# generic-ebpf/generic-ebpf

Hardware: AMD Instinct MI355X
Metric: Mpkt/s device-resident (64-insn filter, 64B pkts); achieved HBM GB/s vs peak (higher is better)
Workload: dtype u64; 1 GPU; c4; desc=64-insn classify + array-map lookup, 64 B packets, packets_total=67108864, packets_per_gpu=67108864, packet_bytes=64, prog_slots=553, dprog_entries=122, variant=0, exec=compiled, kernel_layout=staged64, parallelism=dp1, launch=eager, faulted_packets=0

## Files before the change

generic-ebpf_amd/csrc/asm/gen_interp.py:

```python
#!/usr/bin/env python3
import re
import sys
from typing import NamedTuple

from gen_emit import *
from gen_handlers import handler_body
from gen_image import IMAGES, SETTINGS
from gen_jit import entry_reads, jit_templates
from gen_routines import routines


def kernel(img, name, staged, jit=False):
    k = "K%s%s" % ("s" if staged else "g", "j" if jit else "")
    L = [".globl %s" % name, ".p2align 8", ".type %s,@function" % name, "%s:" % name]
    if name == "ebpf_jit_s64" and img.phased and img.slots == 16:
        L += [".globl ebpf_jit_s64w", ".type ebpf_jit_s64w,@function", "ebpf_jit_s64w:"]
    L += ["v_readfirstlane_b32 %s, v0" % s(S_WAVE),
          "s_lshr_b32 %s, %s, 6" % (s(S_WAVE), s(S_WAVE)),
          "s_load_dwordx16 s[%d:%d], %s" % (S_PROG, S_PROG + 15, karg_regs(
              ("prog", S_PROG), ("maps", S_MAPS), ("data", S_DATA), ("offsets", S_OFFS),
              ("off_base", S_OFFBASE), ("ret", S_RET), ("faults", S_FAULTS), ("hist", S_HIST))),
          "s_load_dwordx8 s[%d:%d], %s" % (S_COUNT, S_COUNT + 7, karg_regs(
              ("count", S_COUNT), ("stride", S_STRIDE), ("start", S_START), ("nmaps", S_NMAPS),
              ("nentries", S_NENT), ("stack_stride", S_STKSTRIDE), ("lds_stack_base", S_LDSBASE))),
          "s_load_dword %s, %s" % (s(S_GSTRIDE), karg("total_waves")),
          "s_load_dword %s, %s" % (s(S_PKTLDS), karg("lds_pkt_base")),
          "s_mov_b64 %s, src_shared_base" % sp(S_SHARED),
          "v_mov_b32 v%d, 0x00010203" % V_SEL,
          "s_getpc_b64 %s" % sp(S_CB),
          ".L%s_pc:" % k,
          "s_add_u32 %s, %s, .Lcb-.L%s_pc" % (s(S_CB), s(S_CB), k),
          "s_addc_u32 %s, %s, 0" % (s(S_CB + 1), s(S_CB + 1)),
          "v_mbcnt_lo_u32_b32 %s, -1, 0" % v(H[0]),
          "v_mbcnt_hi_u32_b32 %s, -1, %s" % (v(H[0]), v(H[0])),
          "v_lshlrev_b32 v%d, 4, %s" % (V_L16, v(H[0])),
          "s_mov_b32 %s, -1" % s(S_PREVG),
          "s_waitcnt lgkmcnt(0)",
          "s_mov_b32 %s, %d" % (s(S_MODE), (staged << MODE_STAGED) | (jit << MODE_JIT)),
          "s_load_dword %s, %s" % (s(S_T3), karg("vflags"))] + (
          ["s_load_dword %s, %s" % (s(S_WPHASE), karg("wphase")) if staged else
           "s_mov_b32 %s, 0" % s(S_WPHASE),
           "s_mov_b32 %s, 0" % s(S_PEND)] if img.phased else []) + [
          "s_waitcnt lgkmcnt(0)",
          "s_bitcmp1_b32 %s, %d" % (s(S_T3), VF_OVERLAY),
          "s_cbranch_scc0 .L%s_noovl" % k,
          mode_set(MODE_OVERLAY),
          ".L%s_noovl:" % k,
          "s_bitcmp1_b32 %s, %d" % (s(S_T3), VF_EXTENTS),
          "s_cbranch_scc0 .L%s_noext" % k,
          mode_set(MODE_EXTENTS),
          ".L%s_noext:" % k]
    if staged:
        L += ["s_bitcmp1_b32 %s, %d" % (s(S_T3), VF_KEEP),
              "s_cbranch_scc0 .L%s_nokeep" % k,
              mode_set(MODE_KEEP),
              ".L%s_nokeep:" % k]
    if not staged:
        L += ["s_bitcmp1_b32 %s, %d" % (s(S_PKTLDS), PKTLDS_HDRSTAGE),
              "s_cbranch_scc0 .L%s_nogs" % k,
              mode_set(MODE_HDRSTAGE),
              ".L%s_nogs:" % k,
              "s_bitcmp1_b32 %s, %d" % (s(S_PKTLDS), PKTLDS_HDRKEEP),
              "s_cbranch_scc0 .L%s_nohl" % k,
              mode_set(MODE_KEEP),
              ".L%s_nohl:" % k,
              "s_and_b32 %s, %s, 0x%x" % (s(S_PKTLDS), s(S_PKTLDS), (1 << PKTLDS_HDRKEEP) - 1)]
    L += ["s_branch .Lprologue"]
    return L


def pkt_setup(idx, tag):
    return ["s_mov_b64 %s, exec" % sp(S_MASK),
            "s_cmp_eq_u64 %s, 0" % sp(S_OFFS),
            "s_cbranch_scc0 .Lps_offsets_%s" % tag,
            "v_mov_b32 %s, %s" % (v(H[1]), s(S_STRIDE)),
            "v_mad_u64_u32 v[%d:%d], %s, v%d, %s, %s" % (V_PKT, V_PKT + 1, sp(S_JUNK), idx,
                                                         v(H[1]), sp(S_DATA)),
            "v_mov_b32 v%d, %s" % (V_LEN, s(S_STRIDE)),
            "s_branch .Lps_stage_%s" % tag,
            ".Lps_offsets_%s:" % tag,
            mode_test(MODE_EXTENTS),
            "s_cselect_b32 %s, 16, 8" % s(S_JUNK),
            "v_mov_b32 %s, %s" % (v(H[1]), s(S_JUNK)),
            "v_mad_u64_u32 %s, %s, v%d, %s, %s" % (vp(H[4]), sp(S_JUNK), idx, v(H[1]), sp(S_OFFS)),
            "global_load_dwordx2 %s, %s, off offset:8" % (vp(R[0]), vp(H[4])),
            "global_load_dwordx2 %s, %s, off" % (vp(H[4]), vp(H[4])),
            "s_waitcnt vmcnt(0)",
            "v_sub_co_u32 v%d, vcc, %s, %s" % (V_LEN, v(R[0]), v(H[4])),
            "v_subb_co_u32 %s, vcc, %s, %s, vcc" % (v(R[1]), v(R[1]), v(H[5])),
            "v_cmp_ne_u32_e32 vcc, 0, %s" % v(R[1]),
            "v_cndmask_b32 v%d, v%d, 0, vcc" % (V_LEN, V_LEN),
            "v_mov_b32 %s, %s" % (v(R[2]), s(S_OFFBASE + 1)),
            "v_sub_co_u32 %s, vcc, %s, %s" % (v(H[4]), v(H[4]), s(S_OFFBASE)),
            "v_subb_co_u32 %s, vcc, %s, %s, vcc" % (v(H[5]), v(H[5]), v(R[2])),
            "v_lshl_add_u64 v[%d:%d], %s, 0, %s" % (V_PKT, V_PKT + 1, vp(H[4]), sp(S_DATA)),
            ] + [
            ".Lps_stage_%s:" % tag,
            mode_test(MODE_HDRSTAGE),
            "s_cbranch_scc0 .Lps_done_%s" % tag,
            "v_cmp_lt_u32_e64 vcc, 63, v%d" % V_LEN,
            "s_and_b64 exec, %s, vcc" % sp(S_MASK),
            "s_cbranch_execz .Lps_done_%s" % tag] + [
            "global_load_dwordx4 v[%d:%d], v[%d:%d], off offset:%d" % (PKT0 + 4 * q, PKT0 + 4 * q + 3,
                                                                       V_PKT, V_PKT + 1, 16 * q)
            for q in range(4)] + [
            "s_waitcnt vmcnt(0)",
            mode_test(MODE_KEEP),
            "s_cbranch_scc0 .Lps_done_%s" % tag,
            "v_mbcnt_lo_u32_b32 %s, -1, 0" % v(H[1]),
            "v_mbcnt_hi_u32_b32 %s, -1, %s" % (v(H[1]), v(H[1])),
            "v_lshl_add_u32 %s, %s, 2, %s" % (v(H[1]), v(H[1]), s(S_PKTLDS))] + lds_pkt_dwords(v(H[1])) + [
            ".Lps_done_%s:" % tag,
            "s_mov_b64 exec, %s" % sp(S_MASK)]


def slot_commit(img):
    if img.retk == 1:
        return []
    L = ["s_mov_b64 exec, -1",
         "s_and_b32 %s, %s, %s" % (s(S_BYTES), s(S_GROUP), s(S_KMASK))]
    if img.phased and img.slots == 16:
        L += ["s_cmp_eq_u32 %s, 0" % s(S_BYTES),
              "s_cbranch_scc0 .Lsc_half",
              "s_bitcmp1_b32 %s, %d" % (s(S_WPHASE), WPHASE_WIDE),
              "s_cbranch_scc0 .Lsc_half",
              "s_xor_b32 %s, %s, 0x80000000" % (s(S_PEND), s(S_PEND)),
              ".Lsc_half:",
              "s_lshr_b32 %s, %s, 28" % (s(S_T0), s(S_PEND)),
              "s_and_b32 %s, %s, 8" % (s(S_T0), s(S_T0)),
              "s_or_b32 %s, %s, %s" % (s(S_BYTES), s(S_BYTES), s(S_T0)),
              "s_bitset1_b32 %s, %s" % (s(S_PEND), s(S_BYTES))]
    elif img.phased:
        L.append("s_bitset1_b32 %s, %s" % (s(S_PEND), s(S_BYTES)))
    return L + [
            "s_lshl_b32 %s, %s, 1" % (s(S_BYTES), s(S_BYTES)),
            "s_set_gpr_idx_on %s, gpr_idx(DST)" % s(S_BYTES),
            "v_mov_b32 v%d, v%d" % (img.v_rb, V_RES),
            "v_mov_b32 v%d, v%d" % (img.v_rb + 1, V_RES + 1),
            "s_set_gpr_idx_off"]


def store_phased(img, tag, final):
    P = s(S_PEND)
    L = ["s_cmp_eq_u32 %s, 0" % s(S_WPHASE),
         "s_cbranch_scc1 .Lph_off_%s" % tag] + (
        ["s_waitcnt lgkmcnt(0)"] if not final else []) + [
         "s_and_b32 %s, %s, 0xffff" % (s(S_T0), P),
         "s_cbranch_scc0 .Lsp_none_%s" % tag]
    if not final:
        L += [
              "s_and_b32 %s, %s, %s" % (s(S_T0), s(S_GROUP), s(S_KMASK)),
              "s_lshr_b32 %s, %s, 28" % (s(S_T1), P),
              "s_and_b32 %s, %s, 8" % (s(S_T1), s(S_T1)),
              "s_cmp_eq_u32 %s, 0" % s(S_T0),
              "s_cbranch_scc0 .Lph_nf_%s" % tag,
              "s_bitcmp1_b32 %s, %d" % (s(S_WPHASE), WPHASE_WIDE),
              "s_cbranch_scc0 .Lph_nf_%s" % tag,
              "s_xor_b32 %s, %s, 8" % (s(S_T1), s(S_T1)),
              ".Lph_nf_%s:" % tag,
              "s_or_b32 %s, %s, %s" % (s(S_T0), s(S_T0), s(S_T1)),
              "s_bitcmp1_b32 %s, %s" % (P, s(S_T0)),
              "s_cbranch_scc1 .Lph_write_%s" % tag,
              "s_and_b32 %s, %s, 0x%x" % (s(S_T1), s(S_WPHASE), 0x1f << WPHASE_PERIOD_SHIFT),
              "s_and_b32 %s, %s, 0xffff" % (s(S_T2), s(S_WPHASE)),
              "s_bfe_u32 %s, %s, %s" % (s(S_T0), s(S_CLOCK), s(S_T1)),
              "s_cmp_lt_u32 %s, %s" % (s(S_T0), s(S_T2)),
              "s_cbranch_scc0 .Lsp_none_%s" % tag,
              ".Lph_write_%s:" % tag]
    L += ["s_mov_b64 exec, -1",
          "v_lshrrev_b32 %s, 1, v%d" % (v(R[0]), V_L16),
          "s_andn2_b32 %s, %s, %s" % (s(S_T1), s(S_PREVG), s(S_KMASK)),
          "s_add_u32 %s, %s, %s" % (s(S_T2), s(S_GSTRIDE), s(S_KMASK)),
          "s_sub_u32 %s, %s, %s" % (s(S_T0), s(S_T1), s(S_T2)),
          "s_bitcmp1_b32 %s, %d" % (s(S_WPHASE), WPHASE_WIDE),
          "s_cselect_b32 %s, %s, 0" % (s(S_T2), s(S_T2)),
          "s_sub_u32 %s, %s, %s" % (s(S_T2), s(S_T0), s(S_T2)),
          "s_and_b32 %s, %s, %s" % (s(S_T3), s(S_PREVG), s(S_KMASK)),
          "s_lshr_b32 s66, %s, 6" % s(S_COUNT),
          "s_add_u32 s67, %s, %s" % (s(S_T1), s(S_KMASK)),
          "s_cmp_lt_u32 s67, s66",
          "s_cbranch_scc0 .Lph_ragged_%s" % tag]
    for lo, g in ((60, S_T1), (62, S_T0), (64, S_T2)):
        L += ["s_lshl_b32 s%d, %s, 9" % (lo, s(g)),
              "s_lshr_b32 s%d, %s, 23" % (lo + 1, s(g)),
              "s_add_u32 s%d, s%d, %s" % (lo, lo, s(S_RET)),
              "s_addc_u32 s%d, s%d, %s" % (lo + 1, lo + 1, s(S_RET + 1))]
    halves = [0] if img.retk == img.slots else [0, 1]

    def slots_of(half, ragged):
        out = []
        for own in (True, False):
            h = half if own else 1 - half
            if h not in halves:
                continue
            for i in range(img.retk):
                j = 8 * h + i
                sk = ".Lph_%s%d_%d_%s" % ("r" if ragged else "f", half, j, tag)
                out += ["s_bitcmp1_b32 %s, %d" % (P, j), "s_cbranch_scc0 %s" % sk]
                if not ragged:
                    if own:
                        out += ["s_cmp_ge_u32 %s, %d" % (s(S_T3), i),
                                "s_cselect_b64 s[66:67], s[60:61], s[64:65]"]
                    out.append("global_store_dwordx2 %s, v[%d:%d], s[%d:%d] offset:%d%s" % (
                        v(R[0]), img.v_rb + 2 * j, img.v_rb + 2 * j + 1, 66 if own else 62,
                        67 if own else 63, 512 * i, SETTINGS.st_policy))
                else:
                    if own:
                        out += ["s_cmp_ge_u32 %s, %d" % (s(S_T3), i),
                                "s_cselect_b32 %s, %s, %s" % (s(S_BYTES), s(S_T1), s(S_T2))]
                    else:
                        out.append("s_mov_b32 %s, %s" % (s(S_BYTES), s(S_T0)))
                    out += ["s_add_u32 %s, %s, %d" % (s(S_BYTES), s(S_BYTES), i),
                            "s_lshl_b32 s66, %s, 6" % s(S_BYTES),
                            "s_sub_u32 s66, %s, s66" % s(S_COUNT),
                            "v_cmp_gt_u32_e64 vcc, s66, %s" % v(R[1]),
                            "s_mov_b64 exec, vcc",
                            "s_lshl_b32 s66, %s, 9" % s(S_BYTES),
                            "s_lshr_b32 s67, %s, 23" % s(S_BYTES),
                            "s_add_u32 s66, s66, %s" % s(S_RET),
                            "s_addc_u32 s67, s67, %s" % s(S_RET + 1),
                            "global_store_dwordx2 %s, v[%d:%d], s[66:67]%s" % (
                                v(R[0]), img.v_rb + 2 * j, img.v_rb + 2 * j + 1, SETTINGS.st_policy),
                            "s_mov_b64 exec, -1"]
                out.append(sk + ":")
        return out

    for ragged in (False, True):
        if ragged:
            L += [".Lph_ragged_%s:" % tag,
                  "v_lshrrev_b32 %s, 4, v%d" % (v(R[1]), V_L16)]
        if len(halves) > 1:
            L += ["s_bitcmp1_b32 %s, 31" % P,
                  "s_cbranch_scc1 .Lph_%sh1_%s" % ("r" if ragged else "f", tag)]
        L += slots_of(0, ragged) + ["s_branch .Lph_done_%s" % tag]
        if len(halves) > 1:
            L += [".Lph_%sh1_%s:" % ("r" if ragged else "f", tag)] + slots_of(1, ragged) + [
                  "s_branch .Lph_done_%s" % tag]
    L += [".Lph_done_%s:" % tag,
          "s_and_b32 %s, %s, 0x80000000" % (P, P),
          "s_branch .Lsp_none_%s" % tag,
          ".Lph_off_%s:" % tag]
    return L


def store_prev_results(img, tag, final):
    L = store_phased(img, tag, final) if img.phased else []
    L += ["s_cmp_eq_u32 %s, -1" % s(S_PREVG),
         "s_cbranch_scc1 .Lsp_none_%s" % tag]
    if not final and img.retk > 1:
        L += ["s_and_b32 %s, %s, %s" % (s(S_T0), s(S_PREVG), s(S_KMASK)),
              "s_cmp_lg_u32 %s, %s" % (s(S_T0), s(S_KMASK)),
              "s_cbranch_scc1 .Lsp_none_%s" % tag]
    L += ["s_mov_b64 exec, -1",
          "s_andn2_b32 %s, %s, %s" % (s(S_T0), s(S_PREVG), s(S_KMASK)) if img.retk > 1 else
          "s_mov_b32 %s, %s" % (s(S_T0), s(S_PREVG)),
          ] + (["v_lshrrev_b32 %s, 4, v%d" % (v(R[1]), V_L16),
                "v_lshl_add_u32 %s, %s, 6, %s" % (v(R[1]), s(S_T0), v(R[1]))] if img.staged else
               ["v_mov_b32 %s, v%d" % (v(R[1]), V_IDX)]) + [
          "v_lshlrev_b32 %s, 3, %s" % (v(R[0]), v(R[1]))]
    for k in range(img.retk):
        if k:
            L += ["s_cmp_lt_u32 %s, %d" % (s(S_KMASK), k),
                  "s_cbranch_scc1 .Lsp_none_%s" % tag,
                  "v_add_u32 %s, 64, %s" % (v(R[1]), v(R[1]))]
        L += ["v_cmp_gt_u32_e64 vcc, %s, %s" % (s(S_COUNT), v(R[1])),
              "s_mov_b64 exec, vcc",
              "global_store_dwordx2 %s, v[%d:%d], %s offset:%d%s" % (
                  v(R[0]), img.v_rb + 2 * k, img.v_rb + 2 * k + 1, sp(S_RET), 512 * k, SETTINGS.st_policy)]
    L.append(".Lsp_none_%s:" % tag)
    return L


def next_group(dst):
    return ["s_and_b32 %s, %s, %s" % (s(dst), s(S_GROUP), s(S_KMASK)),
            "s_cmp_eq_u32 %s, %s" % (s(dst), s(S_KMASK)),
            "s_cselect_b32 %s, %s, 1" % (s(dst), s(S_GSTRIDE)),
            "s_add_u32 %s, %s, %s" % (s(dst), s(dst), s(S_GROUP))]


def common_group_code(img):
    L = [".Lcb:",
         "ebpf_cb:",
         ".Lprologue:"]
    L += ["s_lshl_b32 %s, %s, 6" % (s(S_T0), s(S_WAVE)),
          "v_add_u32 %s, %s, %s" % (v(H[1]), s(S_T0), v(H[0])),
          "v_mul_lo_u32 %s, %s, %s" % (v(H[4]), v(H[1]), s(S_STKSTRIDE)),
          "v_add_u32 v%d, %s, %s" % (V_STK, s(S_LDSBASE), v(H[4]))]
    L += ["v_lshlrev_b32 %s, 2, %s" % (v(H[2]), v(H[1])),
          "v_mov_b32 %s, 0" % v(H[3]),
          "ds_write_b32 %s, %s" % (v(H[2]), v(H[3]))]
    L += ["v_lshlrev_b32 %s, 2, %s" % (v(H[4]), v(H[1])),
          "s_mov_b32 %s, 0" % s(S_T2),
          ".Lmc_loop:",
          "s_cmp_ge_u32 %s, %s" % (s(S_T2), s(S_NMAPS)),
          "s_cbranch_scc1 .Lmc_done",
          "s_lshl_b32 %s, %s, 5" % (s(S_T3), s(S_T2)),
          "s_load_dwordx8 s[%d:%d], %s, %s" % (S_REC, S_REC + 7, sp(S_MAPS), s(S_T3)),
          "s_waitcnt lgkmcnt(0)",
          "s_add_u32 %s, %s, 1" % (s(S_T2), s(S_T2)),
          "s_cmp_eq_u32 s70, -1",
          "s_cbranch_scc1 .Lmc_loop",
          "s_mul_i32 %s, s68, s69" % s(S_T1),
          "s_mov_b32 %s, 0" % s(S_T0),
          ".Lmc_chunk:",
          "s_cmp_ge_u32 %s, %s" % (s(S_T0), s(S_T1)),
          "s_cbranch_scc1 .Lmc_zero",
          "v_add_u32 %s, %s, %s" % (v(H[5]), s(S_T0), v(H[4])),
          "v_cmp_gt_u32_e64 vcc, %s, %s" % (s(S_T1), v(H[5])),
          "s_mov_b64 exec, vcc",
          "global_load_dword %s, %s, s[66:67]" % (v(H[3]), v(H[5])),
          "s_waitcnt vmcnt(0)",
          "v_add_u32 %s, s70, %s" % (v(H[5]), v(H[5])),
          "ds_write_b32 %s, %s" % (v(H[5]), v(H[3])),
          "s_mov_b64 exec, -1",
          "s_add_u32 %s, %s, 1024" % (s(S_T0), s(S_T0)),
          "s_branch .Lmc_chunk",
          ".Lmc_zero:",
          "s_bitcmp1_b32 s71, 29",
          "s_cbranch_scc0 .Lmc_loop",
          "s_and_b32 %s, s71, 0xffff" % s(S_T3),
          "v_mov_b32 %s, 0" % v(H[3]),
          "s_mov_b32 %s, 0" % s(S_T0),
          ".Lmc_zchunk:",
          "s_cmp_ge_u32 %s, %s" % (s(S_T0), s(S_T1)),
          "s_cbranch_scc1 .Lmc_loop",
          "v_add_u32 %s, %s, %s" % (v(H[5]), s(S_T0), v(H[4])),
          "v_cmp_gt_u32_e64 vcc, %s, %s" % (s(S_T1), v(H[5])),
          "s_mov_b64 exec, vcc",
          "v_add_u32 %s, %s, %s" % (v(H[5]), s(S_T3), v(H[5])),
          "ds_write_b32 %s, %s" % (v(H[5]), v(H[3])),
          "s_mov_b64 exec, -1",
          "s_add_u32 %s, %s, 1024" % (s(S_T0), s(S_T0)),
          "s_branch .Lmc_zchunk",
          ".Lmc_done:",
          "s_waitcnt lgkmcnt(0)",
          "s_barrier"]
    L += ["s_add_u32 %s, %s, 63" % (s(S_NGROUPS), s(S_COUNT)),
          "s_lshr_b32 %s, %s, 6" % (s(S_NGROUPS), s(S_NGROUPS)),
          "s_lshl_b32 %s, s2, 2" % s(S_GROUP),
          "s_add_u32 %s, %s, %s" % (s(S_GROUP), s(S_GROUP), s(S_WAVE)),
          "s_lshr_b32 %s, %s, %d" % (s(S_T1), s(S_GSTRIDE), WAVES_SB_SHIFT),
          "s_and_b32 %s, %s, 0xffff" % (s(S_GSTRIDE), s(S_GSTRIDE)),
          "s_lshl_b32 %s, 1, %s" % (s(S_KMASK), s(S_T1)),
          "s_sub_u32 %s, %s, 1" % (s(S_KMASK), s(S_KMASK)),
          "s_lshl_b32 %s, %s, %s" % (s(S_GROUP), s(S_GROUP), s(S_T1)),
          ] + [
          "s_lshl_b32 %s, %s, %s" % (s(S_GSTRIDE), s(S_GSTRIDE), s(S_T1)),
          "s_sub_u32 %s, %s, %s" % (s(S_GSTRIDE), s(S_GSTRIDE), s(S_KMASK)),
          "s_lshl_b32 %s, %s, 12" % (s(S_T0), s(S_WAVE)),
          "s_add_u32 %s, %s, %s" % (s(S_PKTLDS), s(S_PKTLDS), s(S_T0)),
          mode_test(MODE_STAGED),
          "s_cbranch_scc0 .Lgroup_check",
          "s_mov_b32 %s, %s" % (s(S_T0), s(S_GROUP))] + call(".Lr_prefetch") + [
          "s_branch .Lgroup_check"]
    L += [".Lgroup_done:"]
    L += slot_commit(img) + next_group(S_T0) + [
          "s_and_b32 %s, %s, 0x%x" % (s(S_BYTES), s(S_MODE), 1 << MODE_KEEP | 1 << MODE_STAGED),
          "s_cmp_eq_u32 %s, 0x4001" % s(S_BYTES),
          "s_cbranch_scc0 .Lgd_nokeep"] + call(".Lr_prefetch") + [
          ".Lgd_nokeep:",
          "s_mov_b32 %s, %s" % (s(S_GROUP), s(S_T0)),
          ".Lgroup_check:",
          "s_mov_b64 exec, -1",
          "s_cmp_lt_u32 %s, %s" % (s(S_GROUP), s(S_NGROUPS)),
          "s_cbranch_scc0 .Lfinish",
          ] + (
          ["s_cmp_eq_u32 %s, 0" % s(S_WPHASE),
           "s_cbranch_scc1 .Lgc_noclock",
           "s_memrealtime s[%d:%d]" % (S_CLOCK, S_CLOCK + 1),
           ".Lgc_noclock:"] if img.phased else []) + lane_index(img, H[0]) + [
          "v_lshl_add_u32 v%d, %s, 6, %s" % (V_GIDX, s(S_GROUP), v(H[0])),
          "v_cmp_gt_u32_e64 %s, %s, v%d" % (sp(S_ALIVE), s(S_COUNT), V_GIDX),
          ] + [
          mode_test(MODE_STAGED),
          "s_cbranch_scc0 .Lgs_general",
          "s_waitcnt vmcnt(0)",
          "v_and_b32 %s, 0x300, v%d" % (v(H[1]), V_L16),
          "v_mad_u32_u24 %s, %s, 3, v%d" % (v(H[1]), v(H[1]), V_L16),
          "v_add_u32 %s, %s, %s" % (v(H[1]), s(S_PKTLDS), v(H[1]))]
    for q in range(4):
        L.append("ds_read_b128 v[%d:%d], %s offset:%d" % (PKT0 + 4 * q, PKT0 + 4 * q + 3,
                                                          v(H[1]), 256 * q))
    L += ["s_waitcnt lgkmcnt(0)",
          mode_test(MODE_KEEP),
          "s_cbranch_scc0 .Lgs_pf_dma",
          "v_lshrrev_b32 %s, 2, v%d" % (v(H[1]), V_L16),
          "v_add_u32 %s, %s, %s" % (v(H[1]), s(S_PKTLDS), v(H[1]))] + lds_pkt_dwords(v(H[1])) + [
          "s_branch .Lgs_pf_done",
          ".Lgs_pf_dma:"] + next_group(S_T0) + [
          "s_lshr_b32 %s, %s, 6" % (s(S_BYTES), s(S_COUNT)),
          "s_cmp_lt_u32 %s, %s" % (s(S_T0), s(S_BYTES)),
          "s_cbranch_scc0 .Lgs_pf_slow",
          "s_lshr_b32 s65, %s, 20" % s(S_T0),
          "s_lshl_b32 s64, %s, 12" % s(S_T0),
          "s_add_u32 s64, s64, %s" % s(S_DATA),
          "s_addc_u32 s65, s65, %s" % s(S_DATA + 1),
          "s_mov_b64 exec, -1"] + dma_lane_offsets(v(H[4]), v(H[5])) + [
          "s_mov_b32 m0, %s" % s(S_PKTLDS),
          "s_nop 0"] + [
          "global_load_lds_dwordx4 %s, s[64:65] offset:%d%s" % (v(H[4]), 1024 * qq, SETTINGS.ld_policy)
          for qq in range(4)] + [
          "s_branch .Lgs_pf_done",
          ".Lgs_pf_slow:"] + call(".Lr_prefetch") + [
          ".Lgs_pf_done:",
          mode_test(MODE_JIT),
          "s_cbranch_scc1 .Lgs_init",
          "s_mov_b64 exec, %s" % sp(S_ALIVE),
          "v_mov_b32 %s, 64" % v(H[1]),
          "v_mad_u64_u32 v[%d:%d], %s, v%d, %s, %s" % (V_PKT, V_PKT + 1, sp(S_JUNK), V_GIDX,
                                                       v(H[1]), sp(S_DATA)),
          "v_mov_b32 v%d, 64" % V_LEN,
          "s_branch .Lgs_init",
          ".Lgs_general:",
          "s_mov_b64 exec, %s" % sp(S_ALIVE)] + pkt_setup(V_GIDX, "g") + [
          ".Lgs_init:"] + store_prev_results(img, "g", False) + [
          "s_mov_b32 %s, %s" % (s(S_PREVG), s(S_GROUP))] + ([] if img.staged else [
          "s_mov_b64 exec, -1",
          "v_mov_b32 v%d, v%d" % (V_IDX, V_GIDX)]) + [
          "s_mov_b64 exec, %s" % sp(S_ALIVE),
          "s_cmp_eq_u64 %s, 0" % sp(S_FAULTS),
          "s_cbranch_scc1 .Lgs_nofz",
          ] + lane_pkt_index(img, R[9]) + [
          "v_mov_b32 %s, 0" % v(R[8]),
          "global_store_byte %s, %s, %s" % (v(R[9]), v(R[8]), sp(S_FAULTS)),
          ".Lgs_nofz:",
          mode_test(MODE_JIT),
          "s_cbranch_scc0 .Lgs_interp"] + goto("ebpf_jit_area+%d" % JIT_ENTRY_OFF) + [
          ".Lgs_interp:"]
    for r in range(0, 20, 2):
        if r != 2:
            L.append("v_mov_b64 v[%d:%d], 0" % (r, r + 1))
    L += ["v_mov_b64 v[2:3], v[%d:%d]" % (V_PKT, V_PKT + 1),
          "v_add_u32 v20, %s, v%d" % (s(S_STKSTRIDE), V_STK),
          "v_mov_b32 v21, %s" % s(S_SHARED + 1),
          "s_lshl_b32 %s, %s, 5" % (s(S_T0), s(S_START)),
          "v_mov_b32 v%d, %s" % (V_T, s(S_T0))] + goto(".Lr_schedule")
    HR = HIST_REPLICA_BYTES
    L += [".Lfinish:"] + store_prev_results(img, "f", True)
    L += [".Lfinish_body:",
          "s_mov_b64 exec, -1",
          "s_waitcnt vmcnt(0) lgkmcnt(0)",
          "s_barrier"]
    L += lane_index(img, H[0]) + [
          "s_lshl_b32 %s, %s, 6" % (s(S_T0), s(S_WAVE)),
          "v_add_u32 %s, %s, %s" % (v(H[1]), s(S_T0), v(H[0])),
          "s_mov_b32 %s, 0" % s(S_T2),
          ".Lfd_loop:",
          "s_cmp_ge_u32 %s, %s" % (s(S_T2), s(S_NMAPS)),
          "s_cbranch_scc1 .Lfd_done",
          "s_lshl_b32 %s, %s, 5" % (s(S_T3), s(S_T2)),
          "s_load_dwordx8 s[%d:%d], %s, %s" % (S_REC, S_REC + 7, sp(S_MAPS), s(S_T3)),
          "s_waitcnt lgkmcnt(0)",
          "s_add_u32 %s, %s, 1" % (s(S_T2), s(S_T2)),
          "s_bitcmp1_b32 s71, 29",
          "s_cbranch_scc0 .Lfd_loop",
          "s_mul_i32 %s, s68, s69" % s(S_T1),
          "s_add_u32 %s, %s, 63" % (s(S_BYTES), s(S_T1)),
          "s_and_b32 %s, %s, -64" % (s(S_BYTES), s(S_BYTES)),
          "s_add_u32 s66, s66, %s" % s(S_BYTES),
          "s_addc_u32 s67, s67, 0",
          "s_and_b32 %s, s71, 0xffff" % s(S_T3),
          "s_bitcmp1_b32 s71, 28",
          "s_cselect_b32 %s, 3, 2" % s(S_CODE),
          "v_lshlrev_b32 %s, %s, %s" % (v(H[2]), s(S_CODE), v(H[1])),
          "s_lshl_b32 %s, 256, %s" % (s(S_BYTES), s(S_CODE)),
          ".Lfd_word:",
          "v_cmp_gt_u32_e64 vcc, %s, %s" % (s(S_T1), v(H[2])),
          "s_and_saveexec_b64 %s, vcc" % sp(S_MASK),
          "s_cbranch_execz .Lfd_next",
          "v_add_u32 %s, %s, %s" % (v(H[3]), s(S_T3), v(H[2])),
          "v_mov_b32 %s, 0" % v(R[3]),
          "s_cmp_eq_u32 %s, 3" % s(S_CODE),
          "s_cbranch_scc0 .Lfd_r4",
          "ds_read_b64 %s, %s" % (vp(R[2]), v(H[3])),
          "s_branch .Lfd_r",
          ".Lfd_r4:",
          "ds_read_b32 %s, %s" % (v(R[2]), v(H[3])),
          ".Lfd_r:",
          "s_waitcnt lgkmcnt(0)",
          "v_cmp_ne_u64_e64 vcc, 0, %s" % vp(R[2]),
          "s_and_b64 exec, exec, vcc",
          "s_cbranch_execz .Lfd_next",
          "v_mov_b32 %s, %s" % (v(R[0]), v(H[2])),
          "s_cmp_eq_u32 %s, 3" % s(S_CODE),
          "s_cbranch_scc0 .Lfd_w4",
          "global_atomic_add_x2 %s, %s, s[66:67]" % (v(R[0]), vp(R[2])),
          "s_branch .Lfd_next",
          ".Lfd_w4:",
          "global_atomic_add %s, %s, s[66:67]" % (v(R[0]), v(R[2])),
          ".Lfd_next:",
          "s_mov_b64 exec, %s" % sp(S_MASK),
          "v_add_u32 %s, %s, %s" % (v(H[2]), s(S_BYTES), v(H[2])),
          "v_cmp_gt_u32_e64 vcc, %s, %s" % (s(S_T1), v(H[2])),
          "s_and_b64 vcc, vcc, exec",
          "s_cbranch_scc1 .Lfd_word",
          "s_mov_b64 exec, -1",
          "s_branch .Lfd_loop",
          ".Lfd_done:",
          "s_mov_b64 exec, -1",
          "s_cmp_eq_u64 %s, 0" % sp(S_HIST),
          "s_cbranch_scc1 .Lfin_end",
          ] + lane_index(img, H[0]) + [
          "s_lshl_b32 %s, %s, 6" % (s(S_T0), s(S_WAVE)),
          "v_add_u32 %s, %s, %s" % (v(H[1]), s(S_T0), v(H[0])),
          "v_lshlrev_b32 %s, 2, %s" % (v(H[2]), v(H[1])),
          "ds_read_b32 %s, %s" % (v(H[3]), v(H[2])),
          "s_load_dwordx2 %s, %s" % (sp(S_REC), karg("hist_rows")),
          "s_load_dwordx4 s[68:71], %s" % karg("hist_user", "hist_flags", "nwg"),
          "s_waitcnt lgkmcnt(0)",
          "s_cmp_eq_u64 %s, 0" % sp(S_REC),
          "s_cbranch_scc1 .Lfin_atomic",
          "s_and_b32 %s, s2, 7" % s(S_T1),
          "s_mul_i32 %s, %s, %d" % (s(S_T1), s(S_T1), HR),
          "v_lshlrev_b32 %s, 3, %s" % (v(R[0]), v(H[1])),
          "v_add_u32 %s, %s, %s" % (v(R[0]), s(S_T1), v(R[0])),
          "v_mov_b32 %s, %s" % (v(R[2]), v(H[3])),
          "v_mov_b32 %s, 0" % v(R[3]),
          "v_cmp_ne_u32_e64 vcc, 0, %s" % v(H[3]),
          "s_and_saveexec_b64 %s, vcc" % sp(S_SAVE),
          "s_cbranch_execz .Lfin_noadd",
          "global_atomic_add_x2 %s, %s, %s" % (v(R[0]), vp(R[2]), sp(S_REC)),
          ".Lfin_noadd:",
          "s_mov_b64 exec, -1",
          "s_waitcnt vmcnt(0)",
          "s_barrier",
          "s_cmp_eq_u32 %s, 0" % s(S_WAVE),
          "s_cbranch_scc0 .Lfin_flag",
          "s_mov_b64 exec, 1",
          "s_and_b32 %s, s2, 7" % s(S_T1),
          "s_lshl_b32 %s, %s, 6" % (s(S_T0), s(S_T1)),
          "s_add_u32 %s, %s, %d" % (s(S_T0), s(S_T0), HIST_TICKET_OFF),
          "v_mov_b32 %s, %s" % (v(R[4]), s(S_T0)),
          "v_mov_b32 %s, 1" % v(R[5]),
          "global_atomic_add %s, %s, %s, %s sc0" % (v(R[6]), v(R[4]), v(R[5]), sp(S_REC)),
          "s_sub_u32 %s, s71, 1" % s(S_T3),
          "s_sub_u32 %s, %s, %s" % (s(S_T3), s(S_T3), s(S_T1)),
          "s_lshr_b32 %s, %s, 3" % (s(S_T3), s(S_T3)),
          "s_waitcnt vmcnt(0)",
          "v_readfirstlane_b32 %s, %s" % (s(S_T2), v(R[6])),
          "s_cmp_eq_u32 %s, %s" % (s(S_T2), s(S_T3)),
          "s_cselect_b32 %s, 1, 0" % s(S_T2),
          "s_cbranch_scc0 .Lfin_setflag",
          "v_mov_b32 %s, 0" % v(R[10]),
          "global_atomic_swap %s, %s, %s, %s sc0" % (v(R[8]), v(R[4]), v(R[10]), sp(S_REC)),
          "v_mov_b32 %s, %d" % (v(R[9]), HIST_TICKET_OFF + 64 * HIST_REPLICAS),
          "global_atomic_add %s, %s, %s, %s sc0" % (v(R[6]), v(R[9]), v(R[5]), sp(S_REC)),
          "s_min_u32 %s, s71, %d" % (s(S_T3), HIST_REPLICAS),
          "s_sub_u32 %s, %s, 1" % (s(S_T3), s(S_T3)),
          "s_waitcnt vmcnt(0)",
          "v_readfirstlane_b32 %s, %s" % (s(S_T2), v(R[6])),
          "s_cmp_eq_u32 %s, %s" % (s(S_T2), s(S_T3)),
          "s_cselect_b32 %s, 1, 0" % s(S_T2),
          ".Lfin_setflag:",
          "v_mov_b32 %s, %s" % (v(R[7]), s(S_T2)),
          "v_mov_b32 %s, 0" % v(R[8]),
          "ds_write_b32 %s, %s" % (v(R[8]), v(R[7])),
          "s_mov_b64 exec, -1",
          "s_waitcnt lgkmcnt(0)",
          ".Lfin_flag:",
          "s_barrier",
          "v_mov_b32 %s, 0" % v(R[8]),
          "ds_read_b32 %s, %s" % (v(R[7]), v(R[8])),
          "s_waitcnt lgkmcnt(0)",
          "v_readfirstlane_b32 %s, %s" % (s(S_T2), v(R[7])),
          "s_cmp_eq_u32 %s, 0" % s(S_T2),
          "s_cbranch_scc1 .Lfin_end",
          "v_lshlrev_b32 %s, 3, %s" % (v(R[0]), v(H[1])),
          "v_mov_b32 v24, 0",
          "v_mov_b32 v25, 0"]
    for r in range(HIST_REPLICAS):
        L += ["v_add_u32 v%d, %d, %s" % (16 + r, r * HR, v(R[0])),
              "global_atomic_swap_x2 v[%d:%d], v%d, v[24:25], %s sc0" % (2 * r, 2 * r + 1, 16 + r,
                                                                       sp(S_REC))]
    L += ["s_waitcnt vmcnt(0)"]
    for r in range(1, HIST_REPLICAS):
        L += ["v_lshl_add_u64 v[0:1], v[%d:%d], 0, v[0:1]" % (2 * r, 2 * r + 1)]
    L += ["s_bitcmp1_b32 s70, %d" % HIST_STORE,
          "s_cbranch_scc0 .Lfin_add",
          "global_store_dwordx2 %s, v[0:1], s[68:69]" % v(R[0]),
          "s_branch .Lfin_faults",
          ".Lfin_add:",
          "global_atomic_add_x2 %s, v[0:1], s[68:69]" % v(R[0]),
          ".Lfin_faults:",
          "s_cmp_eq_u32 %s, 0" % s(S_WAVE),
          "s_cbranch_scc0 .Lfin_end",
          "s_mov_b64 exec, 1",
          "v_mov_b32 v16, 2048",
          "global_atomic_swap_x2 v[2:3], v16, v[24:25], %s sc0" % sp(S_REC),
          "v_mov_b32 v17, %d" % (HIST_TICKET_OFF + 64 * HIST_REPLICAS),
          "global_atomic_swap v18, v17, v24, %s sc0" % sp(S_REC),
          "s_waitcnt vmcnt(0)",
          "s_bitcmp1_b32 s70, %d" % HIST_STORE,
          "s_cbranch_scc0 .Lfin_fadd",
          "global_store_dwordx2 v16, v[2:3], s[68:69]",
# ... 239 lines not shown
```

generic-ebpf_amd/csrc/host/gpu_runtime.cpp:

```cpp
#include <chrono>

#include "runtime.h"

namespace {

uint32_t
plan_map_lds(const struct ebpf_map *em, uint32_t *used)
{
	if (em->is_hashtable())
		return ~0u;
	const uint64_t bytes = (uint64_t)em->value_size * em->max_entries;
	if (bytes == 0 || bytes % 4 != 0 || *used + bytes > kMapLdsBudget)
		return ~0u;
	const uint32_t off = kMapLdsBase + *used;
	*used += (uint32_t)((bytes + 15) & ~15ull);
	return off;
}

dp_map
map_record(const struct ebpf_map *em, uint32_t *lds_used)
{
	const map_device_layout l = map_device_layout_of(em);
	dp_map m;
	memset(&m, 0, sizeof(m));
	m.handle = (uint64_t)(uintptr_t)em;
	m.value_size = em->value_size;
	m.max_entries = l.slots;
	m.lds_off = plan_map_lds(em, lds_used);
	m.flags = l.flags;
	return m;
}

thread_local std::string t_err;
thread_local int t_dev = 0;
thread_local hipEvent_t t_time_ev[2] = {nullptr, nullptr};
std::atomic<int> g_variant{0};

}

int
fail(int err, const std::string &msg)
{
	t_err = msg;
	return err;
}

int
hip_fail(hipError_t e, const char *what)
{
	return fail(e == hipErrorOutOfMemory ? ENOMEM : EIO,
		    std::string(what) + ": " + hipGetErrorString(e));
}

int
device_count()
{
	int n = 0;
	if (hipGetDeviceCount(&n) != hipSuccess)
		return 0;
	return n;
}

static int
ensure_translated(struct ebpf_prog *ep)
{
	if (ep->xlated)
		return ep->xlated->error;
	auto x = std::make_unique<dprog_host>();
	const auto t0 = std::chrono::steady_clock::now();
	int err = translate_program(ep, *x);
	x->translate_ms =
	    std::chrono::duration<double, std::milli>(std::chrono::steady_clock::now() - t0).count();
	if (err && x->error == 0)
		x->error = err;
	if (!x->error) {
		x->asm_needs_general = asm_program_needs_general(*x);
		x->asm_stores_last = x->asm_needs_general && asm_program_stores_last(*x);
		x->asm_gstage = asm_program_gstage(*x);
		x->asm_pktv = asm_program_hdrlds(*x);
		x->asm_hdrlds = x->asm_pktv && getenv("EBPF_NOHDRLDS") == nullptr;
		x->asm_keep = x->asm_pktv && getenv("EBPF_NOKEEP") == nullptr;
	}
	ep->xlated = std::move(x);
	if (ep->xlated->error)
		return fail(ep->xlated->error, ep->xlated->error_msg);
	return 0;
}

int
prepare(struct ebpf_prog *ep, int device, dprog_device **out)
{
	if (device < 0 || device >= device_count())
		return fail(ENODEV, "no such GPU device");
	std::lock_guard<std::mutex> g(ep->dlock);
	int err = ensure_translated(ep);
	if (err)
		return err;
	if ((int)ep->dev.size() <= device)
		ep->dev.resize(device + 1);
	auto &dp = ep->dev[device];
	if (dp) {
		*out = dp.get();
		return 0;
	}
	hipError_t e = hipSetDevice(device);
	if (e != hipSuccess)
		return hip_fail(e, "hipSetDevice");
	auto nd = std::make_unique<dprog_device>();
	nd->device = device;
	const std::vector<dp_entry> &entries = ep->xlated->entries;
	e = hipMalloc(&nd->d_entries, entries.size() * sizeof(dp_entry));
	if (e != hipSuccess)
		return hip_fail(e, "hipMalloc(program)");
	e = hipMemcpy(nd->d_entries, entries.data(), entries.size() * sizeof(dp_entry),
		      hipMemcpyHostToDevice);
	if (e != hipSuccess)
		return hip_fail(e, "hipMemcpy(program)");
	nd->nentries = (uint32_t)entries.size();
	for (struct ebpf_map *em : ep->xlated->maps) {
		void *mdev = nullptr;
		err = ensure_map_mirror(em, device, &mdev);
		if (err)
			return err;
		dp_map m = map_record(em, &nd->map_lds_bytes);
		m.dev_base = (uint64_t)(uintptr_t)mdev;
		nd->table.push_back(m);
	}
	for (size_t k = 0; k < ep->xlated->atomic_maps.size(); k++) {
		dp_map &m = nd->table[ep->xlated->atomic_maps[k]];
		m.flags |= DP_MAP_ATOMIC | (ep->xlated->atomic_width[k] == 8 ? DP_MAP_ATOMIC64 : 0u);
		const uint32_t bytes = m.value_size * m.max_entries;
		const uint32_t at = (nd->map_lds_bytes + 7) & ~7u;
		if (m.lds_off != ~0u && at + bytes <= kMapLdsBudget && kMapLdsBase + at < 0x10000u) {
			m.flags |= DP_MAP_LDSDELTA | (kMapLdsBase + at);
			nd->map_lds_bytes = at + ((bytes + 15) & ~15u);
		}
	}
	if (!nd->table.empty()) {
		e = hipMalloc(&nd->d_maps, nd->table.size() * sizeof(dp_map));
		if (e != hipSuccess)
			return hip_fail(e, "hipMalloc(map table)");
		e = hipMemcpy(nd->d_maps, nd->table.data(), nd->table.size() * sizeof(dp_map),
			      hipMemcpyHostToDevice);
		if (e != hipSuccess)
			return hip_fail(e, "hipMemcpy(map table)");
	}
	nd->nmaps = (uint32_t)nd->table.size();
	if (prog_writes_maps(*ep->xlated)) {
		const dprog_host &xl = *ep->xlated;
		std::vector<upd_map> um(nd->table.size());
		uint32_t rmax = 8;
		for (size_t t = 0; t < nd->table.size(); t++) {
			um[t].dev_base = nd->table[t].dev_base;
			um[t].value_size = nd->table[t].value_size;
			um[t].max_entries = nd->table[t].max_entries;
			um[t].win_off = nd->win_words;
			um[t].cls = UPD_NONE;
			um[t].gran = nd->table[t].value_size;
			if (in_list(xl.upd_maps, t)) {
				um[t].cls = UPD_DEVICE;
				if (in_list(xl.vstore_maps, t))
					um[t].gran = 1;
				nd->win_words += (uint64_t)nd->table[t].value_size * nd->table[t].max_entries /
						 um[t].gran;
				rmax = std::max(rmax, (nd->table[t].value_size + 7) & ~7u);
			}
			if (in_list(xl.hupd_maps, t)) {
				um[t].cls = UPD_HOST;
				if (nd->table[t].flags & DP_MAP_HASH)
					rmax = std::max(rmax, dp_hash_key_bytes(dp_hash_key_size(nd->table[t].flags)) +
								  ((nd->table[t].value_size + 7) & ~7u));
				else
					rmax = std::max(rmax, (nd->table[t].value_size + 7) & ~7u);
			}
			for (size_t k = 0; k < xl.atomic_maps.size(); k++)
				if (xl.atomic_maps[k] == t) {
					um[t].cls = UPD_ATOMIC;
					um[t].width = xl.atomic_width[k];
				}
		}
		if (xl.vstore_sites)
			rmax = std::max(rmax, DP_REC_VALUE_BYTES - 16);
		nd->upd_stride = 16 + rmax;
		nd->upd_host = um;
		if ((e = hipMalloc(&nd->d_upd, um.size() * sizeof(upd_map))) != hipSuccess ||
		    (e = hipMemcpy(nd->d_upd, um.data(), um.size() * sizeof(upd_map),
				   hipMemcpyHostToDevice)) != hipSuccess)
			return hip_fail(e, "map-write table");
	}
	dp = std::move(nd);
	*out = dp.get();
	return 0;
}

static int
jit_entries(struct ebpf_prog *ep, dprog_device *dp, int mode)
{
	std::lock_guard<std::mutex> g(ep->dlock);
	if (dp->jit_fn[mode])
		return 0;
	if (dp->jit_err[mode])
		return dp->jit_err[mode];
	std::string msg;
	const auto t0 = std::chrono::steady_clock::now();
	int err = asm_jit_build(dp->device, *ep->xlated, mode, dp->table, &dp->jit_mod[mode],
				&dp->jit_fn[mode], mode == 1 ? &dp->jit_fn_wide : nullptr,
				&dp->jit_stride[mode], &msg);
	dp->build_ms[mode] =
	    std::chrono::duration<double, std::milli>(std::chrono::steady_clock::now() - t0).count();
	if (err) {
		dp->jit_err[mode] = err;
		return fail(err, msg);
	}
	return 0;
}

static int
asm_entries(struct ebpf_prog *ep, dprog_device *dp, int mode)
{
	std::lock_guard<std::mutex> g(ep->dlock);
	if (dp->d_asm[mode])
		return 0;
	if (dp->asm_err[mode])
		return dp->asm_err[mode];
	std::string msg;
	const auto t0 = std::chrono::steady_clock::now();
	int err = asm_build_entries(dp->device, *ep->xlated, mode, dp->table, &dp->d_asm[mode],
				    &dp->asm_stride[mode], &msg);
	dp->build_ms[mode] =
	    std::chrono::duration<double, std::milli>(std::chrono::steady_clock::now() - t0).count();
	if (err) {
		dp->asm_err[mode] = err;
		return fail(err, msg);
	}
// ... 351 lines not shown
```

Baseline: 85030 Mpkt/s.

## Batch map-copy loads, hoist prefetch before map staging, merge kernarg waits

Moves the first packet prefetch ahead of the map-to-LDS copy so packet loads overlap the map staging. The map copy now issues up to eight global loads per round before one wait, instead of waiting after each 1 KB chunk. It also merges two kernel-argument load waits into one, drops the vmcnt wait before the final barrier, and caches the getenv lookups. The cost is more VGPRs used in the prologue (v0-v15), plus a risk to correctness if the prefetch's outstanding loads interact with the map-copy vmcnt(0) wait or if dropping the vmcnt wait leaves stores unfinished.

```diff
diff --git a/generic-ebpf_amd/csrc/asm/gen_interp.py b/generic-ebpf_amd/csrc/asm/gen_interp.py
--- a/generic-ebpf_amd/csrc/asm/gen_interp.py
+++ b/generic-ebpf_amd/csrc/asm/gen_interp.py
@@ -25,6 +25,10 @@
               ("nentries", S_NENT), ("stack_stride", S_STKSTRIDE), ("lds_stack_base", S_LDSBASE))),
           "s_load_dword %s, %s" % (s(S_GSTRIDE), karg("total_waves")),
           "s_load_dword %s, %s" % (s(S_PKTLDS), karg("lds_pkt_base")),
+          "s_load_dword %s, %s" % (s(S_T3), karg("vflags"))] + (
+          ["s_load_dword %s, %s" % (s(S_WPHASE), karg("wphase")) if staged else
+           "s_mov_b32 %s, 0" % s(S_WPHASE),
+           "s_mov_b32 %s, 0" % s(S_PEND)] if img.phased else []) + [
           "s_mov_b64 %s, src_shared_base" % sp(S_SHARED),
           "v_mov_b32 v%d, 0x00010203" % V_SEL,
           "s_getpc_b64 %s" % sp(S_CB),
@@ -35,12 +39,7 @@
           "v_mbcnt_hi_u32_b32 %s, -1, %s" % (v(H[0]), v(H[0])),
           "v_lshlrev_b32 v%d, 4, %s" % (V_L16, v(H[0])),
           "s_mov_b32 %s, -1" % s(S_PREVG),
-          "s_waitcnt lgkmcnt(0)",
           "s_mov_b32 %s, %d" % (s(S_MODE), (staged << MODE_STAGED) | (jit << MODE_JIT)),
-          "s_load_dword %s, %s" % (s(S_T3), karg("vflags"))] + (
-          ["s_load_dword %s, %s" % (s(S_WPHASE), karg("wphase")) if staged else
-           "s_mov_b32 %s, 0" % s(S_WPHASE),
-           "s_mov_b32 %s, 0" % s(S_PEND)] if img.phased else []) + [
           "s_waitcnt lgkmcnt(0)",
           "s_bitcmp1_b32 %s, %d" % (s(S_T3), VF_OVERLAY),
           "s_cbranch_scc0 .L%s_noovl" % k,
@@ -278,10 +277,31 @@
             "s_add_u32 %s, %s, %s" % (s(dst), s(dst), s(S_GROUP))]
 
 
+MC_CHUNKS = 8
+
+
 def common_group_code(img):
     L = [".Lcb:",
          "ebpf_cb:",
          ".Lprologue:"]
+    L += ["s_add_u32 %s, %s, 63" % (s(S_NGROUPS), s(S_COUNT)),
+          "s_lshr_b32 %s, %s, 6" % (s(S_NGROUPS), s(S_NGROUPS)),
+          "s_lshl_b32 %s, s2, 2" % s(S_GROUP),
+          "s_add_u32 %s, %s, %s" % (s(S_GROUP), s(S_GROUP), s(S_WAVE)),
+          "s_lshr_b32 %s, %s, %d" % (s(S_T1), s(S_GSTRIDE), WAVES_SB_SHIFT),
+          "s_and_b32 %s, %s, 0xffff" % (s(S_GSTRIDE), s(S_GSTRIDE)),
+          "s_lshl_b32 %s, 1, %s" % (s(S_KMASK), s(S_T1)),
+          "s_sub_u32 %s, %s, 1" % (s(S_KMASK), s(S_KMASK)),
+          "s_lshl_b32 %s, %s, %s" % (s(S_GROUP), s(S_GROUP), s(S_T1)),
+          "s_lshl_b32 %s, %s, %s" % (s(S_GSTRIDE), s(S_GSTRIDE), s(S_T1)),
+          "s_sub_u32 %s, %s, %s" % (s(S_GSTRIDE), s(S_GSTRIDE), s(S_KMASK)),
+          "s_lshl_b32 %s, %s, 12" % (s(S_T0), s(S_WAVE)),
+          "s_add_u32 %s, %s, %s" % (s(S_PKTLDS), s(S_PKTLDS), s(S_T0)),
+          mode_test(MODE_STAGED),
+          "s_cbranch_scc0 .Lpro_nopf",
+          "s_mov_b32 %s, %s" % (s(S_T0), s(S_GROUP))] + call(".Lr_prefetch") + [
+          "s_mov_b64 exec, -1",
+          ".Lpro_nopf:"]
     L += ["s_lshl_b32 %s, %s, 6" % (s(S_T0), s(S_WAVE)),
           "v_add_u32 %s, %s, %s" % (v(H[1]), s(S_T0), v(H[0])),
           "v_mul_lo_u32 %s, %s, %s" % (v(H[4]), v(H[1]), s(S_STKSTRIDE)),
@@ -302,19 +322,33 @@
           "s_cbranch_scc1 .Lmc_loop",
           "s_mul_i32 %s, s68, s69" % s(S_T1),
           "s_mov_b32 %s, 0" % s(S_T0),
-          ".Lmc_chunk:",
+          ".Lmc_round:",
           "s_cmp_ge_u32 %s, %s" % (s(S_T0), s(S_T1)),
-          "s_cbranch_scc1 .Lmc_zero",
-          "v_add_u32 %s, %s, %s" % (v(H[5]), s(S_T0), v(H[4])),
-          "v_cmp_gt_u32_e64 vcc, %s, %s" % (s(S_T1), v(H[5])),
-          "s_mov_b64 exec, vcc",
-          "global_load_dword %s, %s, s[66:67]" % (v(H[3]), v(H[5])),
-          "s_waitcnt vmcnt(0)",
-          "v_add_u32 %s, s70, %s" % (v(H[5]), v(H[5])),
-          "ds_write_b32 %s, %s" % (v(H[5]), v(H[3])),
-          "s_mov_b64 exec, -1",
-          "s_add_u32 %s, %s, 1024" % (s(S_T0), s(S_T0)),
-          "s_branch .Lmc_chunk",
+          "s_cbranch_scc1 .Lmc_zero"]
+    for c in range(MC_CHUNKS):
+        L += (["s_add_u32 %s, %s, %d" % (s(S_BYTES), s(S_T0), 1024 * c),
+               "s_cmp_ge_u32 %s, %s" % (s(S_BYTES), s(S_T1)),
+               "s_cbranch_scc1 .Lmc_issued",
+               "s_mov_b64 exec, -1"] if c else []) + [
+              "v_add_u32 %s, %s, %s" % (v(MC_CHUNKS + c), s(S_BYTES if c else S_T0), v(H[4])),
+              "v_cmp_gt_u32_e64 vcc, %s, %s" % (s(S_T1), v(MC_CHUNKS + c)),
+              "s_mov_b64 exec, vcc",
+              "global_load_dword %s, %s, s[66:67]" % (v(c), v(MC_CHUNKS + c))]
+    L += [".Lmc_issued:",
+          "s_waitcnt vmcnt(0)"]
+    for c in range(MC_CHUNKS):
+        L += (["s_add_u32 %s, %s, %d" % (s(S_BYTES), s(S_T0), 1024 * c),
+               "s_cmp_ge_u32 %s, %s" % (s(S_BYTES), s(S_T1)),
+               "s_cbranch_scc1 .Lmc_written"] if c else []) + [
+              "s_mov_b64 exec, -1",
+              "v_cmp_gt_u32_e64 vcc, %s, %s" % (s(S_T1), v(MC_CHUNKS + c)),
+              "s_mov_b64 exec, vcc",
+              "v_add_u32 %s, s70, %s" % (v(MC_CHUNKS + c), v(MC_CHUNKS + c)),
+              "ds_write_b32 %s, %s" % (v(MC_CHUNKS + c), v(c))]
+    L += [".Lmc_written:",
+          "s_mov_b64 exec, -1",
+          "s_add_u32 %s, %s, %d" % (s(S_T0), s(S_T0), 1024 * MC_CHUNKS),
+          "s_branch .Lmc_round",
           ".Lmc_zero:",
           "s_bitcmp1_b32 s71, 29",
           "s_cbranch_scc0 .Lmc_loop",
@@ -335,24 +369,7 @@
           ".Lmc_done:",
           "s_waitcnt lgkmcnt(0)",
           "s_barrier"]
-    L += ["s_add_u32 %s, %s, 63" % (s(S_NGROUPS), s(S_COUNT)),
-          "s_lshr_b32 %s, %s, 6" % (s(S_NGROUPS), s(S_NGROUPS)),
-          "s_lshl_b32 %s, s2, 2" % s(S_GROUP),
-          "s_add_u32 %s, %s, %s" % (s(S_GROUP), s(S_GROUP), s(S_WAVE)),
-          "s_lshr_b32 %s, %s, %d" % (s(S_T1), s(S_GSTRIDE), WAVES_SB_SHIFT),
-          "s_and_b32 %s, %s, 0xffff" % (s(S_GSTRIDE), s(S_GSTRIDE)),
-          "s_lshl_b32 %s, 1, %s" % (s(S_KMASK), s(S_T1)),
-          "s_sub_u32 %s, %s, 1" % (s(S_KMASK), s(S_KMASK)),
-          "s_lshl_b32 %s, %s, %s" % (s(S_GROUP), s(S_GROUP), s(S_T1)),
-          ] + [
-          "s_lshl_b32 %s, %s, %s" % (s(S_GSTRIDE), s(S_GSTRIDE), s(S_T1)),
-          "s_sub_u32 %s, %s, %s" % (s(S_GSTRIDE), s(S_GSTRIDE), s(S_KMASK)),
-          "s_lshl_b32 %s, %s, 12" % (s(S_T0), s(S_WAVE)),
-          "s_add_u32 %s, %s, %s" % (s(S_PKTLDS), s(S_PKTLDS), s(S_T0)),
-          mode_test(MODE_STAGED),
-          "s_cbranch_scc0 .Lgroup_check",
-          "s_mov_b32 %s, %s" % (s(S_T0), s(S_GROUP))] + call(".Lr_prefetch") + [
-          "s_branch .Lgroup_check"]
+    L += ["s_branch .Lgroup_check"]
     L += [".Lgroup_done:"]
     L += slot_commit(img) + next_group(S_T0) + [
           "s_and_b32 %s, %s, 0x%x" % (s(S_BYTES), s(S_MODE), 1 << MODE_KEEP | 1 << MODE_STAGED),
@@ -439,7 +456,7 @@
     L += [".Lfinish:"] + store_prev_results(img, "f", True)
     L += [".Lfinish_body:",
           "s_mov_b64 exec, -1",
-          "s_waitcnt vmcnt(0) lgkmcnt(0)",
+          "s_waitcnt lgkmcnt(0)",
           "s_barrier"]
     L += lane_index(img, H[0]) + [
           "s_lshl_b32 %s, %s, 6" % (s(S_T0), s(S_WAVE)),
diff --git a/generic-ebpf_amd/csrc/host/gpu_runtime.cpp b/generic-ebpf_amd/csrc/host/gpu_runtime.cpp
--- a/generic-ebpf_amd/csrc/host/gpu_runtime.cpp
+++ b/generic-ebpf_amd/csrc/host/gpu_runtime.cpp
@@ -78,8 +78,10 @@
 		x->asm_stores_last = x->asm_needs_general && asm_program_stores_last(*x);
 		x->asm_gstage = asm_program_gstage(*x);
 		x->asm_pktv = asm_program_hdrlds(*x);
-		x->asm_hdrlds = x->asm_pktv && getenv("EBPF_NOHDRLDS") == nullptr;
-		x->asm_keep = x->asm_pktv && getenv("EBPF_NOKEEP") == nullptr;
+		static const bool no_hdrlds = getenv("EBPF_NOHDRLDS") != nullptr;
+		static const bool no_keep = getenv("EBPF_NOKEEP") != nullptr;
+		x->asm_hdrlds = x->asm_pktv && !no_hdrlds;
+		x->asm_keep = x->asm_pktv && !no_keep;
 	}
 	ep->xlated = std::move(x);
 	if (ep->xlated->error)
```

New measurement: 85160 Mpkt/s (median of 6 runs). Within noise of the previous version (+0.1%).
